# xvyaward/qeft

Hardware: AMD Instinct MI355X
Metric: decode tokens/sec, Llama-2-7B w4 g128 r128 (higher is better)
Workload: dtype f16; 1 GPU; llama-2-7b w4 g128 r128 full decode step, batch 1, greedy, KV context 69..1248 tokens (64-token context + 5 warm-up tokens before the timed region); layers=32, hipgraph=True, parallelism=single GPU

## Files before the change

### include/qeft_hip.h

```cpp
#ifndef QEFT_HIP_H
#define QEFT_HIP_H

#ifdef __cplusplus
extern "C" {
#endif

#define QEFT_OK 0
#define QEFT_ERR_BATCH 1
#define QEFT_ERR_SHAPE 2
#define QEFT_ERR_GROUP 3
#define QEFT_ERR_NULL 4
#define QEFT_ERR_LAUNCH 5
#define QEFT_ERR_ALIGN 6

typedef void* qeft_stream_t;

int qeft_abi_version(void);
const char* qeft_error_string(int code);
int qeft_last_hip_error(void);
const char* qeft_last_variant(void);

int qeft_gemv_w4(const void* x, const void* qweight, const void* scales, const void* scaled_zeros,
                 void* y, int m, int n, int k, int group_size, qeft_stream_t stream);

// ... 78 lines not shown
int qeft_decode_linear(const void* x, const void* qweight, const void* sz_packed, const void* oweight, const void* bias,
                       void* y, int n, int k, int group_size, int n_out, int mode, const void* residual,
                       const float* ssq_in, int n_ssq_in, float eps, const void* gamma_out, void* y_norm, float* ssq_out,
                       qeft_stream_t stream);
int qeft_decode_linear_w3(const void* x, const void* qweight3, const void* sz_packed, const void* oweight, const void* bias,
                          void* y, int n, int k, int group_size, int n_out, int mode, const void* residual,
                          const float* ssq_in, int n_ssq_in, float eps, const void* gamma_out, void* y_norm, float* ssq_out,
                          qeft_stream_t stream);
int qeft_decode_linear_hnorm(const void* h32, const void* gamma_x, const void* qweight, const void* sz_packed, const void* oweight,
                             const void* bias, void* y, int n, int k, int group_size, int n_out, int mode, float eps,
                             qeft_stream_t stream);
long long qeft_gemv_v3_check_extents(int n, int k, int group_size, int n_out, int n_ssq_in, int shrink_rows);
long long qeft_gemv_v3_check_extents_ckpt(int n, int k, int group_size, int n_out, int m, int gather, int shrink_rows);

int qeft_token_begin_norm_blocks(int hidden);
int qeft_token_begin_norm(const void* embed, const void* tok, const void* rope_tab, const int* pos, void* h32, void* rope_row,
                          const void* gamma, void* h_norm, float* ssq_out, int hidden, int vocab, int max_seq,
                          qeft_stream_t stream);
int qeft_rmsnorm_f32(const void* x32, const void* gamma, void* y, int m, int hidden, float eps, qeft_stream_t stream);
int qeft_rope_rows(void* x, const void* cos_tab, const void* sin_tab, int t, int n_heads, int row_stride,
                   qeft_stream_t stream);
int qeft_lm_head_f16(const void* h32, const void* gamma, const void* weight, void* logits, int hidden, int vocab, float eps,
                     qeft_stream_t stream);
int qeft_residual_norm(const void* h32, const void* add, const void* gamma, void* h32_out, void* h_norm, float* ssq_out,
                       int hidden, qeft_stream_t stream);

int qeft_gemm_w3_supported(int m, int n, int k, int group_size, int n_out);
int qeft_gemm_w3(const void* x, const void* qweight3, const void* scales, const void* scaled_zeros, const void* oweight,
                 const void* bias, void* y, int m, int n, int k, int group_size, int n_out, qeft_stream_t stream);
int qeft_gemm_w3_dx_supported(int m, int n, int k, int group_size, int n_out);
int qeft_gemm_w3_dx(const void* dy, const void* qweight3, const void* scales, const void* scaled_zeros, const void* oweight,
                    void* dx, int m, int n, int k, int group_size, int n_out, qeft_stream_t stream);

int qeft_gemv_w3(const void* x, const void* qweight3, const void* scales, const void* scaled_zeros,
                 const void* oweight_il, const void* bias, const void* residual, const void* sz_packed, void* y, int m,
                 int n, int k, int group_size, int n_out, qeft_stream_t stream);
int qeft_gemv_w3_group(const void* x, const void* norm_gamma, float norm_eps, int nparts,
                       const void* const* qweight3, const void* const* scales, const void* const* scaled_zeros,
                       const void* const* oweight_il, const void* const* bias, const void* const* sz_packed,
                       void* const* y, const int* n, int k, int group_size, int n_out, qeft_stream_t stream);
int qeft_gemv_w3_silu(const void* gate, const void* up, const void* qweight3, const void* scales,
                      const void* scaled_zeros, const void* oweight_il, const void* bias, const void* residual,
                      const void* sz_packed, void* y, int n, int k, int group_size, int n_out, qeft_stream_t stream);
int qeft_expand_w3(const void* qweight3, void* qweight4, int n, int k, int n_out, qeft_stream_t stream);

int qeft_token_begin(const void* embed, const void* tok, const void* rope_tab, const int* pos, void* h, void* rope_row,
// ... 76 lines not shown
```

### qeft_amd/_lib.py

```python
import ctypes
import os

import torch

_HERE = os.path.dirname(os.path.abspath(__file__))
LIB_PATH = os.environ.get("QEFT_HIP_LIB") or os.path.join(_HERE, "lib", "libqeft_hip.so")

_p, _i = ctypes.c_void_p, ctypes.c_int

SIGNATURES = {
    "qeft_abi_version": [],
    "qeft_error_string": [_i],
    "qeft_last_hip_error": [],
    "qeft_last_variant": [],
    "qeft_gemv_w4": [_p, _p, _p, _p, _p, _i, _i, _i, _i, _p],
    "qeft_gemv_w4_qeft": [_p, _p, _p, _p, _p, _p, _i, _i, _i, _i, _i, _p],
    "qeft_gemv_w4_fused": [_p, _p, _p, _p, _p, _p, _p, _p, _p, _p, _i, _i, _i, _i, _i, _p],
    "qeft_pack_scales": [_p, _p, _p, _i, _i, _i, _p],
    "qeft_gemm_w4": [_p, _p, _p, _p, _p, _p, _p, _i, _i, _i, _i, _i, _p],
    "qeft_gemm_w4_workspace_bytes": [_i, _i, _i, _i],
    "qeft_gemm_w4_silu_mul": [_p, _p, _p, _p, _p, _p, _p, _p, _i, _i, _i, _i, _i, _p],
    "qeft_gemm_w4_gateup_supported": [_i, _i, _i, _i, _i],
    "qeft_gemm_w4_gateup": [_p, _p, _p, _p, _p, _p, _p, _i, _i, _i, _i, _i, _p],
    "qeft_gemm_w4_ws": [_p, _p, _p, _p, _p, _p, _p, _p, ctypes.c_longlong, _i, _i, _i, _i, _i, _p],
# ... 8 lines not shown
    "qeft_rmsnorm": [_p, _p, _p, _p, _p, _i, _i, ctypes.c_float, _p],
    "qeft_silu_mul": [_p, _p, _p, _i, _p],
    "qeft_gemv_w3": [_p, _p, _p, _p, _p, _p, _p, _p, _p, _i, _i, _i, _i, _i, _p],
    "qeft_gemv_w3_group": [_p, _p, ctypes.c_float, _i, _p, _p, _p, _p, _p, _p, _p, _p, _i, _i, _i, _p],
    "qeft_gemv_w3_silu": [_p, _p, _p, _p, _p, _p, _p, _p, _p, _p, _i, _i, _i, _i, _p],
    "qeft_expand_w3": [_p, _p, _i, _i, _i, _p],
    "qeft_gemm_w3_supported": [_i, _i, _i, _i, _i],
    "qeft_gemm_w3": [_p, _p, _p, _p, _p, _p, _p, _i, _i, _i, _i, _i, _p],
    "qeft_gemm_w3_dx_supported": [_i, _i, _i, _i, _i],
    "qeft_gemm_w3_dx": [_p, _p, _p, _p, _p, _p, _i, _i, _i, _i, _i, _p],
    "qeft_attn_workspace_bytes": [_i, _i],
    "qeft_token_begin": [_p, _p, _p, _p, _p, _p, _i, _i, _i, _p],
    "qeft_token_end": [_p, _p, _p, _i, _i, _p],
    "qeft_decode_linear_blocks": [_i],
    "qeft_decode_linear": [_p, _p, _p, _p, _p, _p, _i, _i, _i, _i, _i, _p, _p, _i, ctypes.c_float, _p, _p, _p, _p],
    "qeft_decode_linear_w3": [_p, _p, _p, _p, _p, _p, _i, _i, _i, _i, _i, _p, _p, _i, ctypes.c_float, _p, _p, _p, _p],
    "qeft_gemv_v3_check_extents": [_i, _i, _i, _i, _i, _i],
    "qeft_gemv_v3_check_extents_ckpt": [_i, _i, _i, _i, _i, _i, _i],
    "qeft_decode_linear_hnorm": [_p, _p, _p, _p, _p, _p, _p, _i, _i, _i, _i, _i, ctypes.c_float, _p],
    "qeft_token_begin_norm_blocks": [_i],
    "qeft_token_begin_norm": [_p, _p, _p, _p, _p, _p, _p, _p, _p, _i, _i, _i, _p],
    "qeft_rmsnorm_f32": [_p, _p, _p, _i, _i, ctypes.c_float, _p],
    "qeft_lm_head_f16": [_p, _p, _p, _p, _i, _i, ctypes.c_float, _p],
    "qeft_rope_rows": [_p, _p, _p, _i, _i, _i, _p],
    "qeft_residual_norm": [_p, _p, _p, _p, _p, _p, _i, _p],
    "qeft_single_query_attention": [_p, _p, _p, _p, _p, _i, _p, _p, _p, _p, _i, _i, _i, _p],
    "qeft_single_query_attention_alibi": [_p, _p, _p, _p, _p, _i, _p, _p, _p, _p, _i, _i, _i, _p, _p],
    "qeft_single_query_attention_generic": [_p, _p, _p, _p, _p, _p, _p, _i, _i, _i, _i, _p, _p],
    "qeft_rope_attn_decode": [_p, _p, _p, _p, _p, _i, _p, _p, _p, _p, _p, _p, _i, _i, _i, _i, _p],
    "qeft_decode_linear_m": [_p, _p, _p, _p, _p, _p, _i, _i, _i, _i, _i, _p, _p, _i, ctypes.c_float, _p, _p, _p, _i, _p],
    "qeft_gemv_v3_check_extents_m": [_i, _i, _i, _i, _i, _i, _i, _i],
    "qeft_token_begin_norm_m": [_p, _p, _p, _p, _p, _p, _p, _p, _p, _i, _i, _i, _i, _p],
    "qeft_attn_m_workspace_bytes": [_i, _i, _i],
    "qeft_rope_attn_decode_m": [_p, _p, _p, _i, _p, _p, _i, _i, _p, _p, _p, _p, _p, _i, _p, _i, _i, _i, _i, _i, _p],
    "qeft_lm_head_f16_m": [_p, _p, _p, _p, _i, _i, ctypes.c_float, _i, _p],
    "qeft_verify_greedy": [_p, _p, _i, _i, _i, _p, _p, _p, _p, _p],
    "qeft_token_begin_norm_batch": [_p, _p, _p, _p, _p, _p, _p, _p, _p, _p, _i, _i, _i, _i, _i, _p],
    "qeft_attn_batch_workspace_bytes": [_i, _i, _i],
    "qeft_rope_attn_decode_batch": [_p, _p, _p, _i, _p, _p, _i, _i, _p, _p, _p, _p, _p, _p, _p, _i, _p, _i, _i, _i, _i, _i, _i, _p],
    "qeft_attn_kv8_workspace_bytes": [_i, _i, _i],
    "qeft_rope_attn_decode_kv8": [_p, _p, _p, _i, _p, _p, _i, _i, _p, _p, _p, _p, _p, _p, _p, _p, _p, _i, _p, _i, _i, _i, _i, _i, _i, _p],
    "qeft_kv8_store_rows": [_p, _p, _i, _p, _p, _p, _p, _i, _i, _i, _i, _p],
    "qeft_attn_m_kv8_workspace_bytes": [_i, _i, _i],
    "qeft_rope_attn_decode_m_kv8": [_p, _p, _p, _i, _p, _p, _i, _i, _p, _p, _p, _p, _p, _p, _p, _i, _p, _i, _i, _i, _i, _i, _p],
    "qeft_attn_prefill": [_p, _i, _p, _p, _i, _p, _i, _i, _i, _i, _i, _p],
    "qeft_attn_prefill_check_extents": [_i, _i, _i, _i, _i, _i, _i],
# ... 58 lines not shown
```

### qeft_amd/csrc/capi.hip

```cpp
#include <hip/hip_runtime.h>

#include <cstdlib>
#include <cstring>
#include <stdint.h>

#include "../../include/qeft_hip.h"
#include "qeft_common.h"
#include "gemv_v3.h"
#include "prefill_attn.h"

namespace qeft {
hipError_t gemv_v3_launch(V3Args a, int mode, hipStream_t st);
int gemv_v3_max_rows(V3Args a, int m_want);
long long gemv_v3_count_out_of_range_ckpt(const V3Geom& G, int n_rows_have, int m, bool gather);
int gemv_v3_blocks(int nsets);
bool gemv_v3_ok(int K, int G, int n_out);
long long gemv_v3_count_out_of_range(const V3Geom& G, int n_rows_have, int n_ssq_in, bool xn, int bits);
hipError_t token_begin_norm_launch(const void* embed, const void* tok, const void* rope_tab, const int* pos, void* h,
                                   void* rope_row, const void* gamma, void* hnorm, float* ssq_out, int hidden, int vocab,
                                   int max_seq, hipStream_t st);
int token_begin_norm_blocks(int hidden);
hipError_t residual_norm_launch(const void* h, const void* add, const void* gamma, void* h_out, void* hnorm, float* ssq_out,
                                int hidden, hipStream_t st);
hipError_t rmsnorm_f32_launch(const void* x, const void* gamma, void* y, int m, int H, float eps, hipStream_t st);
hipError_t rope_rows_launch(void* x, const void* cs, const void* sn, int T, int H, int row_stride, hipStream_t st);
hipError_t lm_head_f16_launch(const void* h32, const void* gamma, const void* W, void* logits, int H, int vocab, float eps,
                              hipStream_t st);
hipError_t gemv_w4_dispatch(const GemvArgs& a, int m, hipStream_t st);
hipError_t gemv_w4_group_dispatch(GemvGroupArgs g, int nparts, hipStream_t st);
hipError_t gemv_w4_silu_dispatch(const GemvArgs& a, hipStream_t st);
hipError_t gemv_w4_smallm_dispatch(const GemvArgs& a, int m, hipStream_t st);
hipError_t gemv_w3_dispatch(const GemvArgs& a, int m, hipStream_t st);
hipError_t gemv_w3_group_dispatch(GemvGroupArgs g, int nparts, hipStream_t st);
hipError_t gemv_w3_silu_dispatch(const GemvArgs& a, hipStream_t st);
hipError_t expand_w3_launch(const void* q3, void* q4, int N, int K, int n_out, hipStream_t st);
hipError_t rmsnorm_launch(const void* x, const void* add, const void* gamma, void* res_out, void* y, int m, int H,
                          float eps, hipStream_t st);
hipError_t silu_mul_launch(const void* gate, const void* up, void* out, int n, hipStream_t st);
hipError_t rope_attn_decode_launch(const void* q, const void* k, const void* v, const void* cs, const void* sn, void* kc,
                                   void* vc, const int* pos, const int* out_pos, void* out, void* ws, int n_heads,
                                   int n_kv, int max_seq, int S, int tab_rows, hipStream_t st, bool k_ft_layout = false,
                                   const float* alibi_slopes = nullptr);
size_t attn_workspace_bytes(int n_heads, int S);
hipError_t sqa_generic_launch(const void* q, const void* k, const void* v, void* kc, void* vc, const int* pos, const float* alibi,
                              void* out, int n_heads, int n_kv, int max_seq, int head_dim, hipStream_t st);
hipError_t token_begin_launch(const void* embed, const void* tok, const void* rope_tab, const int* pos, void* h,
                              void* rope_row, int hidden, int vocab, int max_seq, hipStream_t st);
hipError_t token_end_launch(const void* logits, void* tok, int* pos, int vocab, int greedy, hipStream_t st);
hipError_t gemv_v3_multi_launch(V3Args a, int mode, hipStream_t st);
long long gemv_v3_count_out_of_range_multi(const V3Geom& G, int n_rows_have, int m, int mode, int n_ssq_in);
// ... 579 lines not shown
    if (m < 1 || hidden < 8 || hidden % 8 != 0) return QEFT_ERR_SHAPE;
    if (!x32 || !gamma || !y) return QEFT_ERR_NULL;
    if (!aligned16(x32) || !aligned16(y) || !aligned16(gamma)) return QEFT_ERR_ALIGN;
    return finish(qeft::rmsnorm_f32_launch(x32, gamma, y, m, hidden, eps, (hipStream_t)stream));
}

int qeft_rope_rows(void* x, const void* cos_tab, const void* sin_tab, int t, int n_heads, int row_stride,
                   qeft_stream_t stream) {
    if (t < 1 || n_heads < 1 || row_stride < n_heads * 128) return QEFT_ERR_SHAPE;
    if (!x || !cos_tab || !sin_tab) return QEFT_ERR_NULL;
    return finish(qeft::rope_rows_launch(x, cos_tab, sin_tab, t, n_heads, row_stride, (hipStream_t)stream));
}

int qeft_lm_head_f16(const void* h32, const void* gamma, const void* weight, void* logits, int hidden, int vocab, float eps,
                     qeft_stream_t stream) {
    if (vocab < 1 || hidden < 512 || hidden % 512 != 0) return QEFT_ERR_SHAPE;
    if (!h32 || !gamma || !weight || !logits) return QEFT_ERR_NULL;
    if (!aligned16(h32) || !aligned16(gamma) || !aligned16(weight)) return QEFT_ERR_ALIGN;
    hipError_t e = qeft::lm_head_f16_launch(h32, gamma, weight, logits, hidden, vocab, eps, (hipStream_t)stream);
    if (e == hipErrorInvalidValue) return QEFT_ERR_SHAPE;
    return finish(e);
}

int qeft_silu_mul(const void* gate, const void* up, void* out, int n, qeft_stream_t stream) {
    if (n < 8 || n % 8 != 0) return QEFT_ERR_SHAPE;
    if (!gate || !up || !out) return QEFT_ERR_NULL;
    if (!aligned16(gate) || !aligned16(up) || !aligned16(out)) return QEFT_ERR_ALIGN;
    return finish(qeft::silu_mul_launch(gate, up, out, n, (hipStream_t)stream));
}

void qeft_debug_attn_stamps(void* p) { qeft::g_attn_dbg = (unsigned long long*)p; }

int qeft_attn_workspace_bytes(int n_heads, int n_split) {
    if (n_heads < 1 || n_heads > 4096 || n_split < 1 || n_split > 8) return 0;
    return (int)qeft::attn_workspace_bytes(n_heads, n_split);
}

int qeft_rope_attn_decode(const void* q, const void* k, const void* v, const void* cos_tab, const void* sin_tab,
                          int tab_rows, void* k_cache, void* v_cache, const int* pos, const int* out_pos, void* out,
                          void* workspace, int n_split, int n_heads, int n_kv_heads, int max_seq, qeft_stream_t stream) {
    if (tab_rows != 1 && tab_rows < max_seq) return QEFT_ERR_SHAPE;
    if (n_heads < 1 || n_kv_heads < 1 || n_heads % n_kv_heads != 0 || max_seq < 16 || max_seq % 16 != 0 || max_seq > 32768)
        return QEFT_ERR_SHAPE;
    if (n_split != 1 && n_split != 2 && n_split != 4 && n_split != 8) return QEFT_ERR_SHAPE;
    if (!q || !k || !v || !cos_tab || !sin_tab || !k_cache || !v_cache || !pos || !out) return QEFT_ERR_NULL;
    if (n_split > 1 && !workspace) return QEFT_ERR_NULL;
// ... 463 lines not shown
```

### qeft_amd/csrc/decode_aux.hip

```cpp
#include <cstdlib>

#include "qeft_common.h"
#include "decode_attn.h"

namespace qeft {

__device__ __forceinline__ float block_sum_256(float v, float* sm) {
    v = wave_sum(v);
    const int lane = threadIdx.x & 63, wave = threadIdx.x >> 6;
    __syncthreads();
    if (lane == 0) sm[wave] = v;
    __syncthreads();
    return sm[0] + sm[1] + sm[2] + sm[3];
}

__device__ __forceinline__ float block_max_256(float v, float* sm) {
#pragma unroll
    for (int o = 32; o > 0; o >>= 1) v = fmaxf(v, __shfl_xor(v, o));
    const int lane = threadIdx.x & 63, wave = threadIdx.x >> 6;
    __syncthreads();
    if (lane == 0) sm[wave] = v;
    __syncthreads();
    return fmaxf(fmaxf(sm[0], sm[1]), fmaxf(sm[2], sm[3]));
}

// ... 125 lines not shown
    const size_t base = (size_t)blockIdx.x * H;
    float ss = 0.f;
    for (int i = threadIdx.x; i < H; i += 256) ss += x[base + i] * x[base + i];
    ss = block_sum_256(ss, sm);
    const float rs = rsqrtf(ss / (float)H + eps);
    for (int i = threadIdx.x; i < H; i += 256) y[base + i] = mul_f32_to_f16(x[base + i] * rs, (float)gamma[i]);
}

__global__ __launch_bounds__(256) void rope_rows_kernel(f16* __restrict__ x, const float* __restrict__ cs,
                                                        const float* __restrict__ sn, int H, int row_stride) {
    const int t = blockIdx.x, i = threadIdx.x & 63;
    const float c = cs[(size_t)t * 64 + i], s = sn[(size_t)t * 64 + i];
    for (int h = threadIdx.x >> 6; h < H; h += 4) {
        f16* p = x + (size_t)t * row_stride + h * 128;
        const float a = (float)p[i], b = (float)p[i + 64];
        p[i] = (f16)(a * c - b * s);
        p[i + 64] = (f16)(b * c + a * s);
    }
}

hipError_t rope_rows_launch(void* x, const void* cs, const void* sn, int T, int H, int row_stride, hipStream_t st) {
    hipLaunchKernelGGL(rope_rows_kernel, dim3(T), dim3(256), 0, st, (f16*)x, (const float*)cs, (const float*)sn, H, row_stride);
    return hipGetLastError();
}

template <int LPR>
__global__ __launch_bounds__(512) void lm_head_f16_kernel(const float* __restrict__ h32, const f16* __restrict__ gamma,
                                                          const f16* __restrict__ W, f16* __restrict__ logits, int vocab,
                                                          float eps, int rows_per_block) {
    constexpr int H = 512 * LPR;
    __shared__ float red[8];
    const int tid = threadIdx.x, lane = tid & 63;
    const int wave = __builtin_amdgcn_readfirstlane(tid >> 6);
    float xv[LPR][8];
    float ss = 0.f;
#pragma unroll
    for (int c = 0; c < LPR; ++c) {
        const f32x4 a = *(const f32x4*)(h32 + c * 512 + lane * 8), b = *(const f32x4*)(h32 + c * 512 + lane * 8 + 4);
#pragma unroll
        for (int j = 0; j < 4; ++j) {
            xv[c][j] = a[j];
            xv[c][4 + j] = b[j];
            ss += a[j] * a[j] + b[j] * b[j];
        }
    }
    ss = wave_sum(ss);
// ... 25 lines not shown
            for (int j = 0; j < 4; ++j) acc = __builtin_amdgcn_fdot2(as_h2(cur[c][j]), xh[c][j], acc, false);
        acc = wave_sum(acc);
        if (lane == 0) logits[r] = (f16)acc;
#pragma unroll
        for (int c = 0; c < LPR; ++c) cur[c] = nxt[c];
    }
}

hipError_t lm_head_f16_launch(const void* h32, const void* gamma, const void* W, void* logits, int H, int vocab, float eps,
                              hipStream_t st) {
    const int blocks = vocab >= 4096 ? 512 : (vocab + 7) / 8, rpb = (vocab + blocks - 1) / blocks;
    auto go = [&](auto kern) {
        hipLaunchKernelGGL(kern, dim3(blocks), dim3(512), 0, st, (const float*)h32, (const f16*)gamma, (const f16*)W, (f16*)logits,
                           vocab, eps, rpb);
        return hipGetLastError();
    };
    switch (H) {
        case 512: return go(lm_head_f16_kernel<1>);
        case 1024: return go(lm_head_f16_kernel<2>);
        case 2048: return go(lm_head_f16_kernel<4>);
        case 4096: return go(lm_head_f16_kernel<8>);
        case 5120: return go(lm_head_f16_kernel<10>);
        case 8192: return go(lm_head_f16_kernel<16>);
        default: return hipErrorInvalidValue;
    }
}

__global__ __launch_bounds__(1024) void token_end_kernel(const f16* __restrict__ logits, long long* __restrict__ tok,
                                                         int* __restrict__ pos, int vocab, int greedy) {
    __shared__ float bv[16];
    __shared__ int bi[16];
    const int t = threadIdx.x;
    if (greedy) {
        float best = -INFINITY;
        int idx = 0x7fffffff;
        for (int i = t * 8; i < vocab; i += 1024 * 8) {
            if (i + 8 <= vocab) {
                const h8 v = *(const h8*)(logits + i);
#pragma unroll
                for (int j = 0; j < 8; ++j)
                    if ((float)v[j] > best) { best = (float)v[j]; idx = i + j; }
            } else {
                for (int j = i; j < vocab; ++j)
                    if ((float)logits[j] > best) { best = (float)logits[j]; idx = j; }
            }
        }
// ... 209 lines not shown
```

### qeft_amd/csrc/decode_rows.h

```cpp
#pragma once
#include "qeft_common.h"

namespace qeft {

__device__ __forceinline__ int row_slot(const int* __restrict__ slot_tab, int row, int n_slots) {
    const int s = slot_tab[row];
    return s >= 0 && s < n_slots ? s : -1;
}

__host__ __device__ constexpr size_t attn_b_ctr_floats(int n_heads) { return ((size_t)8 * n_heads + 15) / 16 * 16; }

__host__ __device__ constexpr size_t attn_m_ctr_floats(int n_heads) { return ((size_t)n_heads + 15) / 16 * 16; }

template <class RowPos>
__device__ __forceinline__ void token_begin_norm_row(const f16* __restrict__ embed, const long long* __restrict__ toks,
                                                     const float* __restrict__ rope_tab, float* __restrict__ h,
                                                     float* __restrict__ rope_rows, const f16* __restrict__ gamma,
                                                     f16* __restrict__ hnorm, float* __restrict__ ssq_out, int hidden, int vocab,
                                                     int max_seq, RowPos row_pos) {
    __shared__ float sm[4];
    const int row = blockIdx.y, nb = gridDim.x;
    const long long tk = min(max(toks[row], 0ll), (long long)vocab - 1);
    const int i = (blockIdx.x * 256 + threadIdx.x) * 8;
    float* const hr = h + (size_t)row * hidden;
    float ss = 0.f;
    if (i < hidden) {
        const h8 v = *(const h8*)(embed + (size_t)tk * hidden + i), g = *(const h8*)(gamma + i);
        h8 o;
#pragma unroll
        for (int j = 0; j < 8; ++j) {
            ss += (float)v[j] * (float)v[j];
            o[j] = mul_f32_to_f16((float)v[j], (float)g[j]);
            hr[i + j] = (float)v[j];
        }
        *(h8*)(hnorm + (size_t)row * hidden + i) = o;
    }
    ss = wave_sum(ss);
    const int lane = threadIdx.x & 63, wave = threadIdx.x >> 6;
    if (lane == 0) sm[wave] = ss;
    __syncthreads();
    if (threadIdx.x == 0) ssq_out[(size_t)row * nb + blockIdx.x] = sm[0] + sm[1] + sm[2] + sm[3];
    if (blockIdx.x == 0 && threadIdx.x < 128) {
        const int p = min(max(row_pos(row), 0), max_seq - 1);
        rope_rows[(size_t)row * 128 + threadIdx.x] = rope_tab[(size_t)p * 128 + threadIdx.x];
    }
}

__device__ __forceinline__ int block_argmax_1024(const f16* lg, int vocab, float* bv, int* bi) {
    const int t = threadIdx.x;
    float best = -INFINITY;
    int idx = 0x7fffffff;
    for (int i = t * 8; i < vocab; i += 1024 * 8) {
        if (i + 8 <= vocab && (vocab & 7) == 0) {
            const h8 v = *(const h8*)(lg + i);
#pragma unroll
            for (int j = 0; j < 8; ++j)
                if ((float)v[j] > best) { best = (float)v[j]; idx = i + j; }
        } else {
            for (int j = i; j < min(i + 8, vocab); ++j)
                if ((float)lg[j] > best) { best = (float)lg[j]; idx = j; }
        }
    }
#pragma unroll
    for (int o = 32; o > 0; o >>= 1) {
        const float ob = __shfl_xor(best, o);
        const int oi = __shfl_xor(idx, o);
        if (ob > best || (ob == best && oi < idx)) { best = ob; idx = oi; }
    }
    if ((t & 63) == 0) { bv[t >> 6] = best; bi[t >> 6] = idx; }
    __syncthreads();
// ... 8 lines not shown
```

### qeft_amd/llama.py

```python
import ctypes
import os
import math
import types
from dataclasses import dataclass

import torch
import torch.nn as nn

from . import _lib, fuse, qeft_cuda
from .qlinear import QuantLinear
from .quant import fake_quantize, minmax_params


@dataclass
class LlamaShape:
    hidden: int
    inter: int
    n_layers: int
    n_heads: int
    n_kv_heads: int
    vocab: int
    max_seq: int = 512
    rms_eps: float = 1e-5
    rope_theta: float = 10000.0
# ... 423 lines not shown
        return codes(), codes(), scales(), scales()
    return tuple(torch.zeros(*lead, n_kv, max_seq, 128, dtype=torch.float16, device=dev) for _ in range(2))


def store_kv_rows(lib, k, v, kc, vc, ks, vs, T, start=0):
    if ks is None:
        kc[:, start:start + T] = k.transpose(0, 1)
        vc[:, start:start + T] = v.transpose(0, 1)
        return
    if not (k.stride(2) == 1 and k.stride(1) == 128 and v.stride() == k.stride()):
        k, v = k.contiguous(), v.contiguous()
    _lib.check(lib.qeft_kv8_store_rows(k.data_ptr(), v.data_ptr(), k.stride(0), kc.data_ptr(), vc.data_ptr(), ks.data_ptr(),
                                       vs.data_ptr(), kc.shape[0], kc.shape[1], start, T,
                                       torch.cuda.current_stream(k.device).cuda_stream))


def _ptr_array(tensors):
    arr = (ctypes.c_void_p * len(tensors))()
    for i, t in enumerate(tensors):
        arr[i] = t.data_ptr() if t is not None else None
    return arr


def capture_graph(dev, launch, n, keep):
    cur, side = torch.cuda.current_stream(dev), torch.cuda.Stream(dev)
    saved = [t.clone() for t in keep]

    def restore():
        for t, v in zip(keep, saved):
            t.copy_(v)
    side.wait_stream(cur)
    with torch.cuda.stream(side):
        launch()
    cur.wait_stream(side)
    torch.cuda.synchronize(dev)
    restore()
    graph = torch.cuda.CUDAGraph()
    with torch.cuda.graph(graph):
        for _ in range(n):
            launch()
    restore()
    return graph


def m_row_buffers(eng, M, attn_ws_bytes):
    s, dev = eng.m.shape, eng.dev
    f16, f32 = dict(dtype=torch.float16, device=dev), dict(dtype=torch.float32, device=dev)
    kvd = s.n_kv_heads * s.head_dim
    return types.SimpleNamespace(
        h32=torch.zeros(M, s.hidden, **f32),
        xn=torch.zeros(M, s.hidden, **f16),
        ssq=torch.zeros(M * max(eng.n_ssq_tb, eng.n_ssq_lin) + 4, **f32),
        qkv=torch.zeros(M, s.hidden + 2 * kvd, **f16),
        att=torch.zeros(M, s.hidden, **f16),
        act=torch.zeros(M, s.inter, **f16),
        hn=torch.zeros(M, s.hidden, **f16),
        rope=torch.zeros(M, 128, **f32),
        ws=torch.zeros(max(attn_ws_bytes, 16) // 4, **f32),
        logits=torch.zeros(M, s.vocab, **f16))


class DecodeEngine:

# ... 120 lines not shown
                    self.oneshot.close()
                self.oneshot = None
                self.collective_note = why or "another rank could not build the one-shot collective"
                if collective == "oneshot":
                    raise RuntimeError(f"collective='oneshot' was requested and is not available: {self.collective_note}")
        elif tp and collective == "oneshot":
            raise RuntimeError("collective='oneshot' needs the v3 tensor-parallel path and a real process group")
        if self.tp3:
            self.h32 = torch.zeros(s.hidden, dtype=torch.float32, device=dev)
            self.part32 = torch.zeros(s.hidden, dtype=torch.float32, device=dev)
            self.zero32 = torch.zeros(s.hidden, dtype=torch.float32, device=dev)
            self.n_ssq_tb = self.lib.qeft_token_begin_norm_blocks(s.hidden)
            self.ssq = torch.zeros((self.n_ssq_tb + 3) // 4 * 4, dtype=torch.float32, device=dev)
            self.tp3ops = []
        if self.v3:
            self.h32 = torch.zeros(s.hidden, dtype=torch.float32, device=dev)
            self.n_ssq_tb = self.lib.qeft_token_begin_norm_blocks(s.hidden)
            self.n_ssq_lin = self.lib.qeft_decode_linear_blocks(s.hidden)
            self.ssq = torch.zeros((max(self.n_ssq_tb, self.n_ssq_lin) + 3) // 4 * 4, dtype=torch.float32, device=dev)
            self.qkv_out = torch.zeros(s.hidden + 2 * kvd, **f16)
            self.q, self.k, self.v = self.qkv_out[:s.hidden], self.qkv_out[s.hidden:s.hidden + kvd], self.qkv_out[s.hidden + kvd:]
            self.v3ops = []
            self.row1 = types.SimpleNamespace(h32=self.h32, xn=self.xn, ssq=self.ssq, qkv=self.qkv_out, att=self.att, act=self.act)
        self.lin = []
        self.packs = []
        self.att_pos = []
        for L in model.model.layers:
            names = {nm[0]: ql for nm, ql in layer_linears(L)}
            if self.tp3:
                self.tp3ops.append(self._build_tp3_layer(names))
                continue
            if tp:
                names = {kk: shard_quantlinear(vv, self.rank, P).to(dev) for kk, vv in names.items()}
            self.lin.append(names)
            o = names["o"]
            self.att_pos.append(_inverse_permutation(o.reorder_ids).to(torch.int32).to(dev) if hasattr(o, "reorder_ids") else None)
            qkv = [names["q"], names["k"], names["v"]]
            gu = [names["g"], names["u"]]
            no = s.n_out
            if self.v3:
                self.v3ops.append(dict(qkv=fuse.concat_linears(qkv), o=fuse.single(names["o"]),
                                       gu=fuse.pair_interleave(*gu), d=fuse.single(names["d"])))
            if tp:
                qkv_y = [self.qkv_loc[:self.hs], self.qkv_loc[self.hs:self.hs + self.kvs], self.qkv_loc[self.hs + self.kvs:]]
            else:
                qkv_y = [self.q, self.k, self.v]
# ... 96 lines not shown

    def gemv_kernel_name(self):
        if self.bits == 3 and not self.v3:
            return "qeft::gemv_w4_mfma_group_kernel / gemv_w4_mfma_kernel <BITS = 3>"
        if self.v3 or self.tp3:
            return "qeft::gemv_v3_kernel"
        return "qeft::gemv_w4_mfma_group_kernel / gemv_w4_mfma_kernel"

    def weight_bytes_per_token(self):
        tot = 0
        if self.tp3:
            for ops in self.tp3ops:
                for op in (ops["qkv"], ops["o"], ops["gu"], ops["d"]):
                    n, k, r, g = op.outfeatures, op.infeatures, op.outlierfeatures, op.group_size
                    tot += n * (k - r) // 2 + 2 * (k // g) * n * 2 + n * r * 2 + 2 * k + 2 * n
            return tot
        for names in self.lin:
            for l in names.values():
                n, k, r, g = l.outfeatures, l.infeatures, l.outlierfeatures, l.group_size
                tot += n * (k - r) * l.bits // 8 + 2 * (k // g) * n * 2 + n * r * 2 + 2 * k + 2 * n
        return tot

    @torch.no_grad()
    def _launch_token(self, linears_only=False, only=None):
        self.n_collectives = 0
        if self.v3:
            return self._launch_token_v3(linears_only, only)
        if self.tp3:
            return self._launch_token_tp3(linears_only, only)
        s, lib, ck, P, tp = self.m.shape, self.lib, _lib.check, self.P, self.tp
        w3 = self.bits == 3
        gemv_group = lib.qeft_gemv_w3_group if w3 else lib.qeft_gemv_w4_group
        gemv_silu = lib.qeft_gemv_w3_silu if w3 else lib.qeft_gemv_w4_silu

        def gemv_fused(x, ql, ow, residual, szp, y, n, k, ids=None):
            if w3:
                return lib.qeft_gemv_w3(x, ql.qweight.data_ptr(), ql.scales.data_ptr(), ql.scaled_zeros.data_ptr(), ow,
                                        None, residual, szp, y, 1, n, k, g, no, st)
            return lib.qeft_gemv_w4_fused(x, ql.qweight.data_ptr(), ql.scales.data_ptr(), ql.scaled_zeros.data_ptr(), ow,
                                          None, ids, residual, szp, y, 1, n, k, g, no, st)

        def pick(tag, fn):
            return fn if only in (None, tag) else (lambda *a: 0)
        group_qkv, group_gu = pick("qkv", gemv_group), pick("gu", gemv_group)
        fused_o, fused_d, silu_d = pick("o", gemv_fused), pick("d", gemv_fused), pick("d", gemv_silu)

        st = torch.cuda.current_stream(self.dev).cuda_stream
        h, h2 = self.hbuf
        if not linears_only:
            ck(lib.qeft_token_begin(self.m.model.embed_tokens.weight.data_ptr(), self.tok.data_ptr(),
# ... 67 lines not shown
                                         self.sample_rec.data_ptr(), st))
        else:
            ck(lib.qeft_token_end(self.logits.data_ptr(), self.tok.data_ptr(), self.pos.data_ptr(), s.vocab,
                                  1 if self.greedy else 0, st))

    def _attn(self, li, q, k, v, att_pos, out, st):
        rope = self.rope_row.data_ptr()
        if self.kv_dtype == "fp8":
            _lib.check(self.lib.qeft_rope_attn_decode_kv8(q, k, v, self.heads_l * 128, rope, rope + 64 * 4, 128, 1,
                                                          self.kc[li].data_ptr(), self.vc[li].data_ptr(), self.ks[li].data_ptr(),
                                                          self.vs[li].data_ptr(), self.slot0.data_ptr(), self.pos.data_ptr(), None,
                                                          att_pos.data_ptr() if att_pos is not None else None, out.data_ptr(),
                                                          self.heads_l * 128, self.attn_ws.data_ptr(), self.attn_split, 1,
                                                          self.heads_l, self.kv_heads_l, self.m.shape.max_seq, 1, st))
            return
        _lib.check(self.lib.qeft_rope_attn_decode(q, k, v, rope, rope + 64 * 4, 1, self.kc[li].data_ptr(), self.vc[li].data_ptr(),
                                                  self.pos.data_ptr(), att_pos.data_ptr() if att_pos is not None else None,
                                                  out.data_ptr(), self.attn_ws.data_ptr(), self.attn_split, self.heads_l,
                                                  self.kv_heads_l, self.m.shape.max_seq, st))

    def _head(self, h32, hn, logits, m, st):
        s, lib, ck = self.m.shape, self.lib, _lib.check
        w, gamma = self.m.lm_head.weight, self.m.model.norm.weight.data_ptr()
        if s.hidden in (512, 1024, 2048, 4096, 5120, 8192) and w.dtype == torch.float16 and w.is_contiguous() \
                and os.environ.get("QEFT_LM_HEAD_TORCH") != "1":
            if m is None:
                ck(lib.qeft_lm_head_f16(h32, gamma, w.data_ptr(), logits.data_ptr(), s.hidden, s.vocab, s.rms_eps, st))
            else:
                ck(lib.qeft_lm_head_f16_m(h32, gamma, w.data_ptr(), logits.data_ptr(), s.hidden, s.vocab, s.rms_eps, m, st))
        else:
            ck(lib.qeft_rmsnorm_f32(h32, gamma, hn.data_ptr(), m or 1, s.hidden, s.rms_eps, st))
            if m is None:
                torch.matmul(hn, w.t(), out=logits)
            else:
                torch.matmul(hn[:m], w.t(), out=logits[:m])

    def _token_tail(self, h32, st):
        self._head(h32, self.hn, self.logits, None, st)
        self._token_end(st)

    def _lin_m(self, b, m, st):
        s, lib = self.m.shape, self.lib
        g, no, eps = s.group_size, s.n_out, s.rms_eps
        xn, ssq = b.xn.data_ptr(), b.ssq.data_ptr()

        def lin(op, x, y, mode=0, residual=None, ssq_in=None, n_ssq=0, gamma_out=None):
            return lib.qeft_decode_linear_m(x, op.qweight.data_ptr(), op.sz_packed.data_ptr(), op.oweight.data_ptr() if no else None,
                                            None, y, op.outfeatures, op.infeatures, g, no, mode, residual, ssq_in, n_ssq, eps,
                                            gamma_out, xn if gamma_out else None, ssq if gamma_out else None, m, st)
        return lin

    def _v3_layers(self, b, lin, attn, only=None):
        ck, layers = _lib.check, self.m.model.layers
        xn, ssq, h32 = b.xn.data_ptr(), b.ssq.data_ptr(), b.h32.data_ptr()
        qkv, att, act = b.qkv.data_ptr(), b.att.data_ptr(), b.act.data_ptr()

        lin_qkv, lin_o, lin_gu, lin_d = (lin if only in (None, tag) else (lambda *a, **kw: 0) for tag in ("qkv", "o", "gu", "d"))
        n_ssq = self.n_ssq_tb
        for li, L in enumerate(layers):
            pk = self.v3ops[li]
            ck(lin_qkv(pk["qkv"], xn, qkv, ssq_in=ssq, n_ssq=n_ssq))
            if attn is not None:
                attn(li)
            ck(lin_o(pk["o"], att, h32, residual=h32, gamma_out=L.post_attention_layernorm.weight.data_ptr()))
            n_ssq = self.n_ssq_lin
            ck(lin_gu(pk["gu"], xn, act, mode=1, ssq_in=ssq, n_ssq=n_ssq))
            nxt = layers[li + 1].input_layernorm.weight.data_ptr() if li + 1 < len(layers) else None
            ck(lin_d(pk["d"], act, h32, residual=h32, gamma_out=nxt))

    @torch.no_grad()
    def _launch_token_v3(self, linears_only=False, only=None):
        s, lib, ck, b = self.m.shape, self.lib, _lib.check, self.row1
        st = torch.cuda.current_stream(self.dev).cuda_stream
        g, no, eps = s.group_size, s.n_out, s.rms_eps
        xn, ssq, h32 = b.xn.data_ptr(), b.ssq.data_ptr(), b.h32.data_ptr()
        entry = lib.qeft_decode_linear_w3 if self.bits == 3 else lib.qeft_decode_linear

        def lin(op, x, y, mode=0, residual=None, ssq_in=None, n_ssq=0, gamma_out=None):
            return entry(x, op.qweight.data_ptr(), op.sz_packed.data_ptr(), op.oweight.data_ptr() if no else None, None, y,
                         op.outfeatures, op.infeatures, g, no, mode, residual, ssq_in, n_ssq, eps, gamma_out,
                         xn if gamma_out else None, ssq if gamma_out else None, st)
        if linears_only:
            return self._v3_layers(b, lin, None, only)
        ck(lib.qeft_token_begin_norm(self.m.model.embed_tokens.weight.data_ptr(), self.tok.data_ptr(), self.rope_tab.data_ptr(),
                                     self.pos.data_ptr(), h32, self.rope_row.data_ptr(),
                                     self.m.model.layers[0].input_layernorm.weight.data_ptr(), xn, ssq, s.hidden, s.vocab,
                                     s.max_seq, st))
        q, k, v = self.q.data_ptr(), self.k.data_ptr(), self.v.data_ptr()
        self._v3_layers(b, lin, lambda li: self._attn(li, q, k, v, self.att_pos[li], self.att, st), only)
        self._token_tail(h32, st)

    @torch.no_grad()
    def _launch_token_tp3(self, linears_only=False, only=None):
        s, lib, ck = self.m.shape, self.lib, _lib.check
        st = torch.cuda.current_stream(self.dev).cuda_stream
        g, no, eps = s.group_size, s.n_out, s.rms_eps
        layers = self.m.model.layers
        cur, oth = self.h32, self.part32
        zero = self.zero32.data_ptr()

        def hnorm(op, h, gamma, y, mode=0):
            return lib.qeft_decode_linear_hnorm(h.data_ptr(), gamma.data_ptr(), op.qweight.data_ptr(), op.sz_packed.data_ptr(),
                                                op.oweight.data_ptr() if no else None, None, y, op.outfeatures, op.infeatures, g,
                                                no, mode, eps, st)

        def partial(op, x, h, y):
            return lib.qeft_decode_linear(x, op.qweight.data_ptr(), op.sz_packed.data_ptr(), op.oweight.data_ptr() if no else None,
                                          None, y.data_ptr(), op.outfeatures, op.infeatures, g, no, 0,
                                          h.data_ptr() if self.rank == 0 else zero, None, 0, eps, None, None, None, st)

        def pick(tag, fn):
            return fn if only in (None, tag) else (lambda *a, **kw: 0)
        if not linears_only:
# ... 66 lines not shown
            if g is None:
                g = self.capture(split=sp)
            g.replay()
        else:
            self.attn_split = sp
            self._launch_token()
        self.host_pos += 1

    MULTI = int(os.environ.get("QEFT_MULTI_TOKENS", "8"))

    def run(self, n_tokens):
        assert self.greedy or self.sampling is not None, \
            "run() feeds every token's successor to the next: greedy or sampled decoding only"
        self._check_fresh()
        multi_ok = self.use_graph and os.environ.get("QEFT_MULTI_TOKEN_GRAPH") != "0"
        while n_tokens > 0:
            p, m = self.host_pos, self.MULTI
            sp = self._split_for(p)
            if multi_ok and n_tokens >= m and p + m <= self.m.shape.max_seq and self._split_for(p + m - 1) == sp:
                key = (sp, "sample", m) if self.sampling is not None else (sp, True, m)
                g = self.graphs.get(key)
                if g is None:
                    self.attn_split = sp
                    g = self.graphs[key] = capture_graph(self.dev, self._launch_token, m, (self.pos, self.tok))
                g.replay()
                self.host_pos += m
                n_tokens -= m
            else:
                self.step()
                n_tokens -= 1

    VERIFY_MAX = 8

    def _m_row_unsupported(self):
        if self.tp or self.tp3:
            return "the verify pass runs on the single-GPU engine only (this engine is tensor-parallel)"
        if self.bits != 4:
            return f"the verify pass runs on 4-bit weights only (this engine has {self.bits}-bit weights)"
        if not self.v3:
            return "the verify pass runs on the v3 engine only (QEFT_ENGINE_V2=1, or shapes the v3 GEMV does not take)"
        return None

    def _verify_unsupported(self):
        why = self._m_row_unsupported()
        if why is None and self.kv_dtype != "fp16" and not getattr(self, "kv8_verify", False):
            return (f'the verify pass runs on an fp16 KV cache only (this engine has kv_dtype="{self.kv_dtype}"; '
                    f'build it with kv8_verify=True for the verify pass over an fp8 KV cache)')
# ... 106 lines not shown
```

Measured before the change: 722.1 tokens/s.

## Fuse LM head argmax, token end and next-token begin into one kernel

```diff
diff --git a/include/qeft_hip.h b/include/qeft_hip.h
--- a/include/qeft_hip.h
+++ b/include/qeft_hip.h
@@ -124,6 +124,10 @@
                    qeft_stream_t stream);
 int qeft_lm_head_f16(const void* h32, const void* gamma, const void* weight, void* logits, int hidden, int vocab, float eps,
                      qeft_stream_t stream);
+int qeft_lm_head_turn_workspace_bytes(void);
+int qeft_lm_head_f16_turn(void* h32, const void* gamma, const void* weight, void* logits, int hidden, int vocab, float eps, void* tok,
+                          int* pos, void* workspace, int begin_next, const void* embed, const void* rope_tab, const void* gamma0,
+                          void* h_norm, float* ssq_out, void* rope_row, int max_seq, qeft_stream_t stream);
 int qeft_residual_norm(const void* h32, const void* add, const void* gamma, void* h32_out, void* h_norm, float* ssq_out,
                        int hidden, qeft_stream_t stream);
 
diff --git a/qeft_amd/_lib.py b/qeft_amd/_lib.py
--- a/qeft_amd/_lib.py
+++ b/qeft_amd/_lib.py
@@ -54,6 +54,8 @@
     "qeft_token_begin_norm": [_p, _p, _p, _p, _p, _p, _p, _p, _p, _i, _i, _i, _p],
     "qeft_rmsnorm_f32": [_p, _p, _p, _i, _i, ctypes.c_float, _p],
     "qeft_lm_head_f16": [_p, _p, _p, _p, _i, _i, ctypes.c_float, _p],
+    "qeft_lm_head_turn_workspace_bytes": [],
+    "qeft_lm_head_f16_turn": [_p, _p, _p, _p, _i, _i, ctypes.c_float, _p, _p, _p, _i, _p, _p, _p, _p, _p, _p, _i, _p],
     "qeft_rope_rows": [_p, _p, _p, _i, _i, _i, _p],
     "qeft_residual_norm": [_p, _p, _p, _p, _p, _p, _i, _p],
     "qeft_single_query_attention": [_p, _p, _p, _p, _p, _i, _p, _p, _p, _p, _i, _i, _i, _p],
diff --git a/qeft_amd/csrc/capi.hip b/qeft_amd/csrc/capi.hip
--- a/qeft_amd/csrc/capi.hip
+++ b/qeft_amd/csrc/capi.hip
@@ -26,6 +26,10 @@
 hipError_t rope_rows_launch(void* x, const void* cs, const void* sn, int T, int H, int row_stride, hipStream_t st);
 hipError_t lm_head_f16_launch(const void* h32, const void* gamma, const void* W, void* logits, int H, int vocab, float eps,
                               hipStream_t st);
+hipError_t lm_head_f16_turn_launch(void* h32, const void* gamma, const void* W, void* logits, int H, int vocab, float eps, void* tok,
+                                   int* pos, void* ws, int begin_next, const void* embed, const void* rope_tab, const void* gamma0,
+                                   void* hnorm, float* ssq_out, void* rope_row, int max_seq, hipStream_t st);
+size_t lm_head_turn_workspace_bytes();
 hipError_t gemv_w4_dispatch(const GemvArgs& a, int m, hipStream_t st);
 hipError_t gemv_w4_group_dispatch(GemvGroupArgs g, int nparts, hipStream_t st);
 hipError_t gemv_w4_silu_dispatch(const GemvArgs& a, hipStream_t st);
@@ -651,6 +655,22 @@
     return finish(e);
 }
 
+int qeft_lm_head_turn_workspace_bytes(void) { return (int)qeft::lm_head_turn_workspace_bytes(); }
+
+int qeft_lm_head_f16_turn(void* h32, const void* gamma, const void* weight, void* logits, int hidden, int vocab, float eps, void* tok,
+                          int* pos, void* workspace, int begin_next, const void* embed, const void* rope_tab, const void* gamma0,
+                          void* h_norm, float* ssq_out, void* rope_row, int max_seq, qeft_stream_t stream) {
+    if (vocab < 1 || hidden < 512 || hidden % 512 != 0 || max_seq < 1) return QEFT_ERR_SHAPE;
+    if (!h32 || !gamma || !weight || !logits || !tok || !pos || !workspace) return QEFT_ERR_NULL;
+    if (begin_next && (!embed || !gamma0 || !h_norm || !ssq_out || (rope_row && !rope_tab))) return QEFT_ERR_NULL;
+    if (!aligned16(h32) || !aligned16(gamma) || !aligned16(weight) || !aligned16(workspace)) return QEFT_ERR_ALIGN;
+    if (begin_next && (!aligned16(embed) || !aligned16(gamma0) || !aligned16(h_norm))) return QEFT_ERR_ALIGN;
+    hipError_t e = qeft::lm_head_f16_turn_launch(h32, gamma, weight, logits, hidden, vocab, eps, tok, pos, workspace, begin_next ? 1 : 0,
+                                                 embed, rope_tab, gamma0, h_norm, ssq_out, rope_row, max_seq, (hipStream_t)stream);
+    if (e == hipErrorInvalidValue) return QEFT_ERR_SHAPE;
+    return finish(e);
+}
+
 int qeft_silu_mul(const void* gate, const void* up, void* out, int n, qeft_stream_t stream) {
     if (n < 8 || n % 8 != 0) return QEFT_ERR_SHAPE;
     if (!gate || !up || !out) return QEFT_ERR_NULL;
diff --git a/qeft_amd/csrc/decode_aux.hip b/qeft_amd/csrc/decode_aux.hip
--- a/qeft_amd/csrc/decode_aux.hip
+++ b/qeft_amd/csrc/decode_aux.hip
@@ -1,6 +1,7 @@
 #include <cstdlib>
 
 #include "qeft_common.h"
+#include "decode_rows.h"
 #include "decode_attn.h"
 
 namespace qeft {
@@ -172,6 +173,115 @@
 hipError_t rope_rows_launch(void* x, const void* cs, const void* sn, int T, int H, int row_stride, hipStream_t st) {
     hipLaunchKernelGGL(rope_rows_kernel, dim3(T), dim3(256), 0, st, (f16*)x, (const float*)cs, (const float*)sn, H, row_stride);
     return hipGetLastError();
+}
+
+struct TurnArgs {
+    long long* tok;
+    int* pos;
+    unsigned long long* ws;
+    int begin_next, max_seq, slot_mask;
+    const f16* embed;
+    const float* rope_tab;
+    const f16* gamma0;
+    float* h_out;
+    f16* hnorm;
+    float* ssq_out;
+    float* rope_row;
+};
+constexpr int kTurnSlots = 8, kTurnSlotBytes = 128, kTurnCtrByte = kTurnSlots * kTurnSlotBytes, kTurnWsBytes = kTurnCtrByte + 128;
+
+template <int LPR>
+__global__ __launch_bounds__(512) void lm_head_f16_turn_kernel(const float* h32, const f16* __restrict__ gamma,
+                                                               const f16* __restrict__ W, f16* __restrict__ logits, int vocab,
+                                                               float eps, int rows_per_block, const TurnArgs ta) {
+    constexpr int H = 512 * LPR;
+    const int tid = threadIdx.x, lane = tid & 63;
+    const int wave = __builtin_amdgcn_readfirstlane(tid >> 6);
+    float xv[LPR][8];
+    float ss = 0.f;
+#pragma unroll
+    for (int c = 0; c < LPR; ++c) {
+        const f32x4 a = *(const f32x4*)(h32 + c * 512 + lane * 8), b = *(const f32x4*)(h32 + c * 512 + lane * 8 + 4);
+#pragma unroll
+        for (int j = 0; j < 4; ++j) {
+            xv[c][j] = a[j];
+            xv[c][4 + j] = b[j];
+            ss += a[j] * a[j] + b[j] * b[j];
+        }
+    }
+    ss = wave_sum(ss);
+    const float rs = rsqrtf(ss / (float)H + eps);
+    h2 xh[LPR][4];
+#pragma unroll
+    for (int c = 0; c < LPR; ++c) {
+        const h8 g = *(const h8*)(gamma + c * 512 + lane * 8);
+#pragma unroll
+        for (int j = 0; j < 4; ++j)
+            xh[c][j] = h2{mul_f32_to_f16(xv[c][2 * j] * rs, (float)g[2 * j]), mul_f32_to_f16(xv[c][2 * j + 1] * rs, (float)g[2 * j + 1])};
+    }
+    const int r_end = min(vocab, (int)(blockIdx.x + 1) * rows_per_block);
+    int r = blockIdx.x * rows_per_block + wave;
+    u32x4 cur[LPR], nxt[LPR];
+    auto load_row = [&](int row, u32x4 (&dst)[LPR]) {
+        const u32x4* p = (const u32x4*)(W + (size_t)min(row, vocab - 1) * H) + lane;
+#pragma unroll
+        for (int c = 0; c < LPR; ++c) dst[c] = __builtin_nontemporal_load(p + c * 64);
+    };
+    load_row(r, cur);
+    float best = -INFINITY;
+    int best_r = 0x7fffffff;
+    for (; r < r_end; r += 8) {
+        load_row(r + 8, nxt);
+        float acc = 0.f;
+#pragma unroll
+        for (int c = 0; c < LPR; ++c)
+#pragma unroll
+            for (int j = 0; j < 4; ++j) acc = __builtin_amdgcn_fdot2(as_h2(cur[c][j]), xh[c][j], acc, false);
+        acc = wave_sum(acc);
+        const f16 lg = (f16)acc;
+        if (lane == 0) logits[r] = lg;
+        if ((float)lg > best) { best = (float)lg; best_r = r; }
+#pragma unroll
+        for (int c = 0; c < LPR; ++c) cur[c] = nxt[c];
+    }
+    __shared__ unsigned long long keys[8];
+    __shared__ float sm[8];
+    __shared__ long long s_tok;
+    __shared__ int s_pos;
+    if (lane == 0) keys[wave] = argmax_key(best, best_r);
+    __syncthreads();
+    if (tid == 0) {
+        unsigned long long key = keys[0];
+#pragma unroll
+        for (int w = 1; w < 8; ++w) key = keys[w] > key ? keys[w] : key;
+        if (key) {
+            const unsigned long long was = __hip_atomic_fetch_max(ta.ws + (blockIdx.x & ta.slot_mask) * (kTurnSlotBytes / 8), key,
+                                                                  __ATOMIC_RELAXED, __HIP_MEMORY_SCOPE_AGENT);
+            asm volatile("s_waitcnt vmcnt(0)" ::"v"(was) : "memory");
+        }
+        unsigned* ctr = (unsigned*)((char*)ta.ws + kTurnCtrByte);
+        const unsigned ticket = __hip_atomic_fetch_add(ctr, 1u, __ATOMIC_RELAXED, __HIP_MEMORY_SCOPE_AGENT);
+        int p = -1;
+        if (ticket == gridDim.x - 1) {
+            unsigned long long got[kTurnSlots], top = 0ull;
+#pragma unroll
+            for (int i = 0; i < kTurnSlots; ++i)
+                got[i] = __hip_atomic_exchange(ta.ws + i * (kTurnSlotBytes / 8), 0ull, __ATOMIC_RELAXED, __HIP_MEMORY_SCOPE_AGENT);
+#pragma unroll
+            for (int i = 0; i < kTurnSlots; ++i) top = got[i] > top ? got[i] : top;
+            __hip_atomic_store(ctr, 0u, __ATOMIC_RELAXED, __HIP_MEMORY_SCOPE_AGENT);
+            const long long tk = argmax_key_index(top);
+            p = *ta.pos + 1;
+            *ta.tok = tk;
+            *ta.pos = p;
+            s_tok = min(tk, (long long)vocab - 1);
+            p = min(max(p, 0), ta.max_seq - 1);
+        }
+        s_pos = p;
+    }
+    __syncthreads();
+    if (s_pos < 0 || !ta.begin_next) return;
+    token_begin_norm_512(ta.embed, s_tok, ta.rope_tab, s_pos, ta.h_out, ta.rope_row, ta.gamma0, ta.hnorm, ta.ssq_out, H, sm);
 }
 
 template <int LPR>
@@ -243,6 +353,32 @@
         case 4096: return go(lm_head_f16_kernel<8>);
         case 5120: return go(lm_head_f16_kernel<10>);
         case 8192: return go(lm_head_f16_kernel<16>);
+        default: return hipErrorInvalidValue;
+    }
+}
+
+size_t lm_head_turn_workspace_bytes() { return kTurnWsBytes; }
+
+hipError_t lm_head_f16_turn_launch(void* h32, const void* gamma, const void* W, void* logits, int H, int vocab, float eps, void* tok,
+                                   int* pos, void* ws, int begin_next, const void* embed, const void* rope_tab, const void* gamma0,
+                                   void* hnorm, float* ssq_out, void* rope_row, int max_seq, hipStream_t st) {
+    static const int slots_env = getenv("QEFT_TURN_SLOTS") ? atoi(getenv("QEFT_TURN_SLOTS")) : kTurnSlots;
+    const TurnArgs ta{(long long*)tok, pos, (unsigned long long*)ws, begin_next, max_seq, slots_env == 1 ? 0 : kTurnSlots - 1,
+                      (const f16*)embed, (const float*)rope_tab,
+                      (const f16*)gamma0, (float*)h32, (f16*)hnorm, ssq_out, (float*)rope_row};
+    const int blocks = vocab >= 4096 ? 512 : (vocab + 7) / 8, rpb = (vocab + blocks - 1) / blocks;
+    auto go = [&](auto kern) {
+        hipLaunchKernelGGL(kern, dim3(blocks), dim3(512), 0, st, (const float*)h32, (const f16*)gamma, (const f16*)W, (f16*)logits,
+                           vocab, eps, rpb, ta);
+        return hipGetLastError();
+    };
+    switch (H) {
+        case 512: return go(lm_head_f16_turn_kernel<1>);
+        case 1024: return go(lm_head_f16_turn_kernel<2>);
+        case 2048: return go(lm_head_f16_turn_kernel<4>);
+        case 4096: return go(lm_head_f16_turn_kernel<8>);
+        case 5120: return go(lm_head_f16_turn_kernel<10>);
+        case 8192: return go(lm_head_f16_turn_kernel<16>);
         default: return hipErrorInvalidValue;
     }
 }
diff --git a/qeft_amd/csrc/decode_rows.h b/qeft_amd/csrc/decode_rows.h
--- a/qeft_amd/csrc/decode_rows.h
+++ b/qeft_amd/csrc/decode_rows.h
@@ -46,6 +46,42 @@
     }
 }
 
+__device__ __forceinline__ void token_begin_norm_512(const f16* __restrict__ embed, long long tk, const float* __restrict__ rope_tab,
+                                                     int p, float* h, float* rope_row, const f16* __restrict__ gamma, f16* hnorm,
+                                                     float* ssq_out, int hidden, float* sm) {
+    const int t = threadIdx.x, lane = t & 63, wave = t >> 6;
+    for (int base = 0; base < hidden; base += 4096) {
+        const int i = base + t * 8;
+        float ss = 0.f;
+        if (i < hidden) {
+            const h8 v = *(const h8*)(embed + (size_t)tk * hidden + i), g = *(const h8*)(gamma + i);
+            h8 o;
+#pragma unroll
+            for (int j = 0; j < 8; ++j) {
+                ss += (float)v[j] * (float)v[j];
+                o[j] = mul_f32_to_f16((float)v[j], (float)g[j]);
+                h[i + j] = (float)v[j];
+            }
+            *(h8*)(hnorm + i) = o;
+        }
+        ss = wave_sum(ss);
+        __syncthreads();
+        if (lane == 0) sm[wave] = ss;
+        __syncthreads();
+        const int piece = base / 2048 + (t >> 8);
+        if ((t & 255) == 0 && piece * 2048 < hidden) ssq_out[piece] = sm[wave] + sm[wave + 1] + sm[wave + 2] + sm[wave + 3];
+    }
+    if (t < 128 && rope_row) rope_row[t] = rope_tab[(size_t)p * 128 + t];
+}
+
+__device__ __forceinline__ unsigned long long argmax_key(float best, int idx) {
+    if (idx == 0x7fffffff) return 0ull;
+    uint32_t u = best == 0.f ? 0u : (uint32_t)__builtin_bit_cast(uint16_t, (f16)best);
+    u = (u & 0x8000u) ? (~u & 0xffffu) : (u | 0x8000u);
+    return ((unsigned long long)u << 32) | (uint32_t)~(uint32_t)idx;
+}
+__device__ __forceinline__ long long argmax_key_index(unsigned long long key) { return key ? (long long)(uint32_t)~(uint32_t)key : 0ll; }
+
 __device__ __forceinline__ int block_argmax_1024(const f16* lg, int vocab, float* bv, int* bi) {
     const int t = threadIdx.x;
     float best = -INFINITY;
diff --git a/qeft_amd/llama.py b/qeft_amd/llama.py
--- a/qeft_amd/llama.py
+++ b/qeft_amd/llama.py
@@ -469,7 +469,8 @@
     return arr
 
 
-def capture_graph(dev, launch, n, keep):
+def capture_graph(dev, launch, n, keep, indexed=False):
+    call = launch if indexed else (lambda i: launch())
     cur, side = torch.cuda.current_stream(dev), torch.cuda.Stream(dev)
     saved = [t.clone() for t in keep]
 
@@ -478,14 +479,14 @@
             t.copy_(v)
     side.wait_stream(cur)
     with torch.cuda.stream(side):
-        launch()
+        call(0)
     cur.wait_stream(side)
     torch.cuda.synchronize(dev)
     restore()
     graph = torch.cuda.CUDAGraph()
     with torch.cuda.graph(graph):
-        for _ in range(n):
-            launch()
+        for i in range(n):
+            call(i)
     restore()
     return graph
 
@@ -652,6 +653,8 @@
             self.q, self.k, self.v = self.qkv_out[:s.hidden], self.qkv_out[s.hidden:s.hidden + kvd], self.qkv_out[s.hidden + kvd:]
             self.v3ops = []
             self.row1 = types.SimpleNamespace(h32=self.h32, xn=self.xn, ssq=self.ssq, qkv=self.qkv_out, att=self.att, act=self.act)
+            self.token_turn = os.environ.get("QEFT_TOKEN_TURN") != "0"
+            self.turn_ws = torch.zeros(self.lib.qeft_lm_head_turn_workspace_bytes() // 4, dtype=torch.int32, device=dev)
         self.lin = []
         self.packs = []
         self.att_pos = []
@@ -794,10 +797,10 @@
         return tot
 
     @torch.no_grad()
-    def _launch_token(self, linears_only=False, only=None):
+    def _launch_token(self, linears_only=False, only=None, begun=False, begin_next=False):
         self.n_collectives = 0
         if self.v3:
-            return self._launch_token_v3(linears_only, only)
+            return self._launch_token_v3(linears_only, only, begun, begin_next)
         if self.tp3:
             return self._launch_token_tp3(linears_only, only)
         s, lib, ck, P, tp = self.m.shape, self.lib, _lib.check, self.P, self.tp
@@ -911,8 +914,7 @@
     def _head(self, h32, hn, logits, m, st):
         s, lib, ck = self.m.shape, self.lib, _lib.check
         w, gamma = self.m.lm_head.weight, self.m.model.norm.weight.data_ptr()
-        if s.hidden in (512, 1024, 2048, 4096, 5120, 8192) and w.dtype == torch.float16 and w.is_contiguous() \
-                and os.environ.get("QEFT_LM_HEAD_TORCH") != "1":
+        if self._head_fused_ok():
             if m is None:
                 ck(lib.qeft_lm_head_f16(h32, gamma, w.data_ptr(), logits.data_ptr(), s.hidden, s.vocab, s.rms_eps, st))
             else:
@@ -924,7 +926,24 @@
             else:
                 torch.matmul(hn[:m], w.t(), out=logits[:m])
 
-    def _token_tail(self, h32, st):
+    def _head_fused_ok(self):
+        s, w = self.m.shape, self.m.lm_head.weight
+        return s.hidden in (512, 1024, 2048, 4096, 5120, 8192) and w.dtype == torch.float16 and w.is_contiguous() \
+            and os.environ.get("QEFT_LM_HEAD_TORCH") != "1"
+
+    def _turn_ok(self):
+        return self.v3 and self.token_turn and self.greedy and self.sampling is None and self._head_fused_ok()
+
+    def _token_tail(self, h32, st, begin_next=False):
+        if self._turn_ok():
+            s, m = self.m.shape, self.m
+            _lib.check(self.lib.qeft_lm_head_f16_turn(
+                h32, m.model.norm.weight.data_ptr(), m.lm_head.weight.data_ptr(), self.logits.data_ptr(), s.hidden, s.vocab,
+                s.rms_eps, self.tok.data_ptr(), self.pos.data_ptr(), self.turn_ws.data_ptr(), 1 if begin_next else 0,
+                m.model.embed_tokens.weight.data_ptr(), self.rope_tab.data_ptr(), m.model.layers[0].input_layernorm.weight.data_ptr(),
+                self.row1.xn.data_ptr(), self.row1.ssq.data_ptr(), self.rope_row.data_ptr(), s.max_seq, st))
+            return
+        assert not begin_next
         self._head(h32, self.hn, self.logits, None, st)
         self._token_end(st)
 
@@ -958,7 +977,7 @@
             ck(lin_d(pk["d"], act, h32, residual=h32, gamma_out=nxt))
 
     @torch.no_grad()
-    def _launch_token_v3(self, linears_only=False, only=None):
+    def _launch_token_v3(self, linears_only=False, only=None, begun=False, begin_next=False):
         s, lib, ck, b = self.m.shape, self.lib, _lib.check, self.row1
         st = torch.cuda.current_stream(self.dev).cuda_stream
         g, no, eps = s.group_size, s.n_out, s.rms_eps
@@ -971,13 +990,15 @@
                          xn if gamma_out else None, ssq if gamma_out else None, st)
         if linears_only:
             return self._v3_layers(b, lin, None, only)
-        ck(lib.qeft_token_begin_norm(self.m.model.embed_tokens.weight.data_ptr(), self.tok.data_ptr(), self.rope_tab.data_ptr(),
-                                     self.pos.data_ptr(), h32, self.rope_row.data_ptr(),
-                                     self.m.model.layers[0].input_layernorm.weight.data_ptr(), xn, ssq, s.hidden, s.vocab,
-                                     s.max_seq, st))
+        assert not (begun or begin_next) or self._turn_ok()
+        if not begun:
+            ck(lib.qeft_token_begin_norm(self.m.model.embed_tokens.weight.data_ptr(), self.tok.data_ptr(), self.rope_tab.data_ptr(),
+                                         self.pos.data_ptr(), h32, self.rope_row.data_ptr(),
+                                         self.m.model.layers[0].input_layernorm.weight.data_ptr(), xn, ssq, s.hidden, s.vocab,
+                                         s.max_seq, st))
         q, k, v = self.q.data_ptr(), self.k.data_ptr(), self.v.data_ptr()
         self._v3_layers(b, lin, lambda li: self._attn(li, q, k, v, self.att_pos[li], self.att, st), only)
-        self._token_tail(h32, st)
+        self._token_tail(h32, st, begin_next)
 
     @torch.no_grad()
     def _launch_token_tp3(self, linears_only=False, only=None):
@@ -1090,7 +1111,11 @@
                 g = self.graphs.get(key)
                 if g is None:
                     self.attn_split = sp
-                    g = self.graphs[key] = capture_graph(self.dev, self._launch_token, m, (self.pos, self.tok))
+                    turn = self._turn_ok()
+
+                    def launch(i, turn=turn, m=m):
+                        self._launch_token(begun=turn and i > 0, begin_next=turn and i < m - 1)
+                    g = self.graphs[key] = capture_graph(self.dev, launch, m, (self.pos, self.tok), indexed=True)
                 g.replay()
                 self.host_pos += m
                 n_tokens -= m
```

Measured after the change: 724.3 tokens/s (median of 6 runs). Within noise of the previous version (+0.3%).
